# udaysankar01/xfeatSLAM

Measured on AMD Instinct MI355X. Metric: XFeat frames/s (VGA, 4096 kpts) + 4096x4096 desc-match pairs/s, higher is better.
Workload: dtype f32

## Files before the change

### include/xfeat_hip_bench.h

```cpp
#ifndef XFEAT_HIP_BENCH_H
#define XFEAT_HIP_BENCH_H

#include "xfeat_hip.h"

#ifdef __cplusplus
extern "C" {
#endif

enum {
    XFH_K_NONE = 0, XFH_K_MNN_GEMM = 1, XFH_K_CONV_MFMA = 2, XFH_K_CONV_DIRECT = 3,
    XFH_K_NMS = 4, XFH_K_SELECT = 5, XFH_K_DESC = 6, XFH_K_HEADS = 7, XFH_K_DIST_I32 = 8,
    XFH_K_PREPROC = 9, XFH_K_BEST2 = 10, XFH_K_DISTINCTIVE = 11, XFH_K_MNN_GEMM_SEG = 12,
    XFH_K_GRID_BUILD = 13, XFH_K_SEARCH_WINDOW = 14,
    XFH_K_FRAME_FINISH = 15, XFH_K_PROJ_CANDIDATES = 16, XFH_K_PROJ_RESOLVE = 17, XFH_K_PROJ_COUNT = 18, XFH_K_FUSE_SEARCH = 19,
    XFH_K_TRIANGULATION_SEARCH = 20, XFH_K_BOW_CANDIDATES = 21, XFH_K_BOW_RESOLVE = 22,
    XFH_K_MAPPROJ_CANDIDATES = 23, XFH_K_SIM3_SEARCH = 24, XFH_K_SIM3_AGREE = 25,
    XFH_K_INIT_CANDIDATES = 27, XFH_K_INIT_RESOLVE = 28, XFH_K_INIT_FINAL = 29,
    XFH_K_VOCAB_DESCEND = 31, XFH_K_VOCAB_FINISH = 32, XFH_K_BOWDB_SCORE = 33, XFH_K_BOWDB_SELECT = 34,
    XFH_K_POSE_OPTIMIZE = 35, XFH_K_COUNT = 36
};
int xfh_timing_enable(xfh_ctx* ctx, int kernel_id, unsigned layer_mask);
int xfh_timing_read(xfh_ctx* ctx, int* launches, double* total_ms);
int xfh_bench_mnn_gemm(xfh_ctx* ctx, const void* d_image1, int n1, const void* d_image2, int n2, int iters, double* us_per_launch);
int xfh_bench_match_prepared(xfh_ctx* ctx, const void* d_image1, int n1, const void* d_image2, int n2, float min_cossim,
                             int* d_idx1, int* d_idx2, float* d_dist, int* d_n_matches, int iters, double* us_per_call);
int xfh_bench_match_raw(xfh_ctx* ctx, const float* d_d1, int n1, const float* d_d2, int n2, float min_cossim,
                        int* d_idx1, int* d_idx2, float* d_dist, int* d_n_matches, int iters, double* us_per_call);
int xfh_bench_mnn_gemm_batch(xfh_ctx* ctx, int n_pairs, const void* const* d_image1, const int* n1, const void* const* d_image2, const int* n2,
                             int iters, double* us_per_launch, double* sclk_mhz);
int xfh_bench_match_batch(xfh_ctx* ctx, int n_pairs, const void* const* d_image1, const int* n1, const void* const* d_image2, const int* n2, float min_cossim,
                          int* const* d_idx1, int* const* d_idx2, float* const* d_dist, int* d_n_matches, int iters, double* us_per_call);
int xfh_debug_match_plan(int n_pairs, const int* n1, const int* n2, int num_cu, int* tiles, int* workgroups, int* tile0, int* planes_max, int* wg_lo,
                         unsigned long long* keys);
const char* xfh_kernel_name(int kernel_id);

enum {
    XFH_T_X = 0, XFH_T_XSTAT = 1, XFH_T_SKIP_POOL = 2,
    XFH_T_FEATS = 6, XFH_T_H1 = 8, XFH_T_K1H = 9,
    XFH_T_RAW0 = 16, XFH_T_STAT0 = 48, XFH_T_SEL = 80
};
int xfh_debug_tensor(xfh_ctx* ctx, int id, int frame, float* out, size_t capacity, size_t* count_out);

int xfh_debug_select(xfh_ctx* ctx, const unsigned long long* keys, int n, int width, int lap0, int lap1, int form,
                     unsigned long long* sel_out, int* n_out, int* hdr_out);


int xfh_bench_calib(xfh_ctx* ctx, int mode, size_t nbytes, int iters);
int xfh_bench_sclk(xfh_ctx* ctx, int mfmas, double* sclk_mhz, double* cycles_per_mfma);

#ifdef __cplusplus
}
#endif
#endif
```

### xfeatslam_amd/capi.py

```python
from __future__ import annotations

import ctypes as C
import os

import numpy as np

_DIR = os.path.dirname(os.path.abspath(__file__))
LIB_PATH = os.environ.get("XFEAT_HIP_LIB") or os.path.join(_DIR, "libxfeat_hip.so")
KNOBS_LIB_PATH = os.path.join(_DIR, "libxfeat_hip_knobs.so")

KP_DTYPE = np.dtype([("x", "<f4"), ("y", "<f4"), ("size", "<f4"), ("angle", "<f4"),
                     ("response", "<f4"), ("octave", "<i4"), ("class_id", "<i4")])
assert KP_DTYPE.itemsize == 28

OK = 0
STATUS = {0: "OK", 1: "INVALID_ARG", 2: "EMPTY_IMAGE", 3: "BAD_SIZE", 4: "NO_WEIGHTS", 5: "BAD_WEIGHTS",
          6: "HIP", 7: "NO_DEVICE", 8: "OUT_OF_MEMORY", 9: "BATCH_TOO_LARGE", 10: "IO", 11: "COMM"}
ERR_EMPTY_IMAGE = 2
ERR_NO_DEVICE = 7
ERR_COMM = 11

K = dict(NONE=0, MNN_GEMM=1, CONV_MFMA=2, CONV_DIRECT=3, NMS=4, SELECT=5, DESC=6, HEADS=7, DIST_I32=8, PREPROC=9, BEST2=10, DISTINCTIVE=11, MNN_GEMM_SEG=12, GRID_BUILD=13, SEARCH_WINDOW=14, FRAME_FINISH=15, PROJ_CANDIDATES=16, PROJ_RESOLVE=17, PROJ_COUNT=18, FUSE_SEARCH=19, TRIANGULATION_SEARCH=20, BOW_CANDIDATES=21, BOW_RESOLVE=22, MAPPROJ_CANDIDATES=23, SIM3_SEARCH=24, SIM3_AGREE=25, INIT_CANDIDATES=27, INIT_RESOLVE=28, INIT_FINAL=29, VOCAB_DESCEND=31, VOCAB_FINISH=32, BOWDB_SCORE=33, BOWDB_SELECT=34, POSE_OPTIMIZE=35)
T = dict(X=0, XSTAT=1, SKIP_POOL=2, FEATS=6, H1=8, K1H=9, RAW0=16, STAT0=48, SEL=80)


class Config(C.Structure):
    _fields_ = [("device", C.c_int32), ("max_height", C.c_int32), ("max_width", C.c_int32),
                ("nfeatures", C.c_int32), ("max_batch", C.c_int32), ("bn_mode", C.c_int32),
                ("nms_threshold", C.c_float), ("flags", C.c_int32), ("reserved", C.c_int32 * 7)]


class GridBounds(C.Structure):
    _fields_ = [("min_x", C.c_float), ("min_y", C.c_float), ("max_x", C.c_float), ("max_y", C.c_float)]


class Camera(C.Structure):
    _fields_ = [("fx", C.c_float), ("fy", C.c_float), ("cx", C.c_float), ("cy", C.c_float), ("k1", C.c_float), ("k2", C.c_float),
                ("p1", C.c_float), ("p2", C.c_float), ("k3", C.c_float), ("bf", C.c_float), ("width", C.c_int32), ("height", C.c_int32),
                ("reserved", C.c_int32 * 4)]


class Sim3Side(C.Structure):
    _fields_ = [("n", C.c_int), ("grid", C.c_void_p), ("kps", C.c_void_p), ("desc", C.c_void_p), ("desc_stride_bytes", C.c_size_t),
                ("points", C.c_void_p), ("dist", C.c_void_p), ("mp_desc", C.c_void_p), ("flags", C.c_void_p), ("Tw", C.c_void_p),
                ("status", C.c_void_p), ("match", C.c_void_p), ("best_dist", C.c_void_p), ("n_window", C.c_void_p), ("n_tested", C.c_void_p),
                ("level", C.c_void_p), ("proj_out", C.c_void_p)]
# ... 278 lines not shown
```

### xfeatslam_amd/csrc/capi_bench.cpp

```cpp
#include "capi_internal.h"
#include "mnn_seg_plan.h"
#include <stdlib.h>

template <typename F>
static int time_calls(xfh_ctx* c, int warmup, int iters, double* us_per_call, F call) {
    hipEvent_t e0, e1;
    HIPCK(c, hipEventCreate(&e0));
    if (hipEventCreate(&e1) != hipSuccess) { hipEventDestroy(e0); return XFH_ERR_HIP; }
    hipError_t e = hipSuccess;
    for (int i = 0; i < warmup && e == hipSuccess; ++i) e = call();
    if (e == hipSuccess) e = hipEventRecord(e0, c->stream);
    for (int i = 0; i < iters && e == hipSuccess; ++i) e = call();
    if (e == hipSuccess) e = hipEventRecord(e1, c->stream);
    if (e == hipSuccess) e = hipEventSynchronize(e1);
    float ms = 0.f;
    if (e == hipSuccess) e = hipEventElapsedTime(&ms, e0, e1);
    hipEventDestroy(e0); hipEventDestroy(e1);
    *us_per_call = (double)ms * 1e3 / iters;
    HIPCK(c, e);
    return XFH_OK;
}

extern "C" {

// ... 71 lines not shown
        tot += ms;
    }
    if (launches) *launches = t.nev;
    if (total_ms) *total_ms = tot;
    const bool overflow = t.dropped > 0;
    t.nev = 0; t.dropped = 0;
    return overflow ? XFH_ERR_BATCH_TOO_LARGE : XFH_OK;
}

int xfh_debug_tensor(xfh_ctx* c, int id, int frame, float* out, size_t cap, size_t* count_out) {
    if (!c || frame < 0 || frame >= c->B || !count_out) return XFH_ERR_INVALID_ARG;
    HIPCK(c, hipStreamSynchronize(c->stream));
    const size_t xs = (size_t)c->Hmax * c->Wmax;
    const int H = c->H, W = c->W, h8 = H / 8, w8 = W / 8, h4 = H / 4, w4 = W / 4;
    const float* src = nullptr; size_t n = 0;
    if (!was_written(c, id)) return XFH_ERR_INVALID_ARG;
    switch (id) {
        case XFH_T_X: src = c->X + frame * xs; n = (size_t)H * W; break;
        case XFH_T_XSTAT: src = c->xstat + frame * 2; n = 2; break;
        case XFH_T_SKIP_POOL: src = c->skip_pool + frame * (xs / 16); n = (size_t)h4 * w4; break;
        case XFH_T_FEATS: src = c->feats + frame * c->raw_stride[17]; n = (size_t)h8 * w8 * 64; break;
        case XFH_T_H1: src = c->H1 + frame * (xs / 64); n = (size_t)h8 * w8; break;
        case XFH_T_K1H: src = c->K1h + frame * xs; n = (size_t)H * W; break;
        default:
            if (id >= XFH_T_RAW0 && id < XFH_T_RAW0 + XFH_NUM_LAYERS) {
                const int i = id - XFH_T_RAW0;
                if (!c->raw[i]) return XFH_ERR_INVALID_ARG;
                src = c->raw[i] + frame * c->raw_stride[i]; n = (size_t)c->lh[i] * c->lw[i] * XFH_LAYERS[i].cout;
            } else if (id >= XFH_T_STAT0 && id < XFH_T_STAT0 + XFH_NUM_LAYERS) {
                const int i = id - XFH_T_STAT0;
                src = c->stat[i] + (size_t)frame * 2 * XFH_LAYERS[i].cout; n = 2 * (size_t)XFH_LAYERS[i].cout;
            } else if (id == XFH_T_SEL) {
                int N = 0;
                HIPCK(c, hipMemcpy(&N, c->sel_n + frame, sizeof(int), hipMemcpyDeviceToHost));
                *count_out = (size_t)N * 3;
                if (!out || cap < (size_t)N * 3) return out ? XFH_ERR_INVALID_ARG : XFH_OK;
                std::vector<u64> keys((size_t)N);
                if (N > 0) HIPCK(c, hipMemcpy(keys.data(), c->sel_key + (size_t)frame * c->cfg.nfeatures, (size_t)N * 8, hipMemcpyDeviceToHost));
                for (int i = 0; i < N; ++i) {
                    const unsigned idx = (unsigned)(keys[i] & 0xFFFFFFFFull);
                    out[i * 3 + 0] = (float)(idx % (unsigned)W); out[i * 3 + 1] = (float)(idx / (unsigned)W);
                    out[i * 3 + 2] = ord2f(~(unsigned)(keys[i] >> 32));
                }
                return XFH_OK;
            } else return XFH_ERR_INVALID_ARG;
    }
// ... 20 lines not shown
```

### xfeatslam_amd/csrc/kernels_conv.hip

```cpp
#include "ctx.h"
#include "heads_kp4.hip.h"
#include <stdlib.h>

struct ConvArgs {
    const float* in;
    StatSrc st;
    size_t in_stride;
    int Hin, Win;
    const float* w;
    const float* bias;
    float* out;
    size_t out_stride;
    int Hout, Wout;
    double* part;
    size_t part_stride;
    int tiles_x;
    const float* pool; size_t pool_stride; const float* skip_w; const float* skip_b;
    const float* r4; size_t s4; int H4, W4; StatSrc st4;
    const float* r5; size_t s5; int H5, W5; StatSrc st5;
    const float* xstat; const float* w0; const float* bias0;
    int dbg;
};

enum { PRO_PLAIN = 0, PRO_BN = 1, PRO_IN = 2, PRO_B2IN = 3, PRO_FUSE = 4, PRO_L0 = 5, PRO_UNFOLD = 6, PRO_FUSEA = 7  };
// ... 1187 lines not shown
    if constexpr (EPI == EPI_STATS) {
        sum += __shfl_xor(sum, 16); sq += __shfl_xor(sq, 16);
        sum += __shfl_xor(sum, 32); sq += __shfl_xor(sq, 32);
        double* s_red = (double*)smem;
        if (q == 0) { s_red[(pg * COUTW + cg * 16 + p) * 2] = sum; s_red[(pg * COUTW + cg * 16 + p) * 2 + 1] = sq; }
        __syncthreads();
        for (int co = t; co < COUTW; co += NTHR) {
            double S = 0.0, SS = 0.0;
#pragma unroll
            for (int m = 0; m < PGY; ++m) { S += s_red[(m * COUTW + co) * 2]; SS += s_red[(m * COUTW + co) * 2 + 1]; }
            double* pp = a.part + (size_t)b * a.part_stride + ((size_t)tile * COUT + co0 + co) * 2;
            pp[0] = S; pp[1] = SS;
        }
    }
    XFH_STAMP(a, 5);
}

enum { MID_BIAS_STORE = 0 , MID_BIAS_RELU = 1  };
struct ChainArgs {
    ConvArgs a;
    const float* w1; const float* bias1;
    const float* w2; const float* bias2;
    float* mid_out; size_t mid_stride;
};
template <int NL, int WM, int PRO, int MID0, int EPI, bool SSTAT = false>
__global__ __launch_bounds__(64 * WM)
void k_chain1x1(ChainArgs ca, int ntile, int total) {
    constexpr int CIN = 64, COUT = 64, NT = 2, WW = 16, WH = 2, TH = WM * WH, TW = WW;
    constexpr int NTHR = 64 * WM, COUTP = 64, CP = CIN + 4, WS = CIN + 4, G = CIN / 8;
    constexpr int NITEM = TH * TW * G, NIT = (NITEM + NTHR - 1) / NTHR;
    constexpr int IN_FLOATS = TH * TW * CP, W_FLOATS = COUTP * WS;
    static_assert(NTHR % G == 0 && NIT <= 32, "staging");
    const ConvArgs& a = ca.a;

    extern __shared__ __attribute__((aligned(16))) float smem[];
    float* s_in = smem;
    float* s_w = smem + IN_FLOATS;
    double* s_red = (double*)(s_w + NL * W_FLOATS);
    float* s_stat = (float*)(s_red + WM * COUTP * 2);
    static_assert(!SSTAT || sizeof(double) * 512 <= sizeof(float) * IN_FLOATS, "bn_fold scratch in the input tile");
    int stat_b = -1;

    const int t = threadIdx.x;
    {
        const float* ws[3] = {a.w, ca.w1, ca.w2};
#pragma unroll
        for (int l = 0; l < NL; ++l)
            for (int f = t; f < COUTP * (CIN / 4); f += NTHR) {
// ... 83 lines not shown
                    for (int j = 0; j < 4; ++j)
                        acc[n] = __builtin_amdgcn_mfma_f32_32x32x2f32(av[j], bv[j], acc[n], 0, 0, 0);
                }
            }
            if (l == NL - 1) break;
            const bool store_mid = l == 0 && MID0 == MID_BIAS_STORE;
            if (store_mid) {
                double dsum[NT], dsq[NT];
                float* wave_out = ca.mid_out + (size_t)b * ca.mid_stride + ((size_t)oy0 * a.Wout + tx0) * COUT;
                conv_epilogue<COUT, NT, WW, WH, EPI_BIAS>(acc, wave_out, a.Wout, a.Hout - oy0, a.Wout - tx0, i, h, bias0, dsum, dsq);
            } else {
                XFH_MFMA_SETTLE();
            }
#pragma unroll
            for (int n = 0; n < NT; ++n) {
                const int c = n * 32 + i;
                const int pos = (c & ~7) + 4 * (c & 1) + ((c & 7) >> 1);
                const float bv = l == 0 ? bias0[n] : bias1[n];
#pragma unroll
                for (int r = 0; r < 16; ++r) {
                    float v = acc[n][r] + bv;
                    if (!store_mid) v = fmaxf(v, 0.f);
                    mid_row[((r & 3) + 8 * (r >> 2)) * CP + pos] = v;
                }
            }
        }

        double sum[NT], sq[NT];
        {
            float* wave_out = a.out + (size_t)b * a.out_stride + ((size_t)oy0 * a.Wout + tx0) * COUT;
            conv_epilogue<COUT, NT, WW, WH, EPI>(acc, wave_out, a.Wout, a.Hout - oy0, a.Wout - tx0, i, h, biasl, sum, sq);
        }
        if constexpr (EPI == EPI_STATS) {
#pragma unroll
            for (int n = 0; n < NT; ++n) {
                sum[n] += __shfl_xor(sum[n], 32);
                sq[n] += __shfl_xor(sq[n], 32);
                if (h == 0) {
                    const int co = n * 32 + i;
                    s_red[(wm * COUTP + co) * 2 + 0] = sum[n];
                    s_red[(wm * COUTP + co) * 2 + 1] = sq[n];
                }
            }
        }
        __syncthreads();
        if constexpr (EPI == EPI_STATS) {
// ... 342 lines not shown
        default: return hipErrorInvalidValue;
    }
}

hipError_t launch_basic_layer(xfh_ctx* c, int li, const float* in, size_t in_stride, int src, int pro, int Hin, int Win, int B) {
    if (c->cfg.bn_mode == XFH_BN_RUNNING_FOLDED) return launch_basic_layer_t<EPI_BIAS_RELU>(c, li, in, in_stride, src, pro, Hin, Win, B);
    return launch_basic_layer_t<EPI_STATS>(c, li, in, in_stride, src, pro, Hin, Win, B);
}

hipError_t launch_block1_stats(xfh_ctx* c, const StatSrc& xs, int H, int W, int B) {
    const int np = conv_layer_npart(0, H, W);
    c->lh[0] = H; c->lw[0] = W; c->npart[0] = np;
    const size_t xsz = (size_t)c->Hmax * c->Wmax;
    launch_k(c, XFH_K_CONV_DIRECT, 0, k_block1_stats, dim3(np, 1, B), dim3(256), 0, (const float*)c->X, xsz, xs, H, W,
             (W + L0S_TW - 1) / L0S_TW, (const float*)c->w.direct[0], c->part[0], c->part_stride[0], c->skip_pool, xsz / 16);
    hipError_t e = hipGetLastError();
    mark_written(c, XFH_T_SKIP_POOL);
    if (e != hipSuccess || consumer_fold(B)) return e;
    hipLaunchKernelGGL(k_bn_finalize, dim3(B), dim3(256), 0, c->stream, (const double*)c->part[0], c->part_stride[0], np, 4, (double)H * (double)W, c->stat[0]);
    mark_written(c, XFH_T_STAT0);
    return hipGetLastError();
}

template <int NL, int WM, int PRO, int MID0, int EPI, bool SSTAT = false>
static hipError_t chain_launch(xfh_ctx* c, const ChainArgs& ca, int B, int* npart_out, int layer) {
    constexpr int TH = 2 * WM, TW = 16;
    constexpr size_t LDS = sizeof(float) * ((size_t)TH * TW * 68 + (size_t)NL * 64 * 68 + (SSTAT ? 128 : 0)) + sizeof(double) * WM * 64 * 2;
    static_assert(LDS <= 160 * 1024, "LDS budget");
    ChainArgs aa = ca;
    aa.a.tiles_x = (ca.a.Wout + TW - 1) / TW;
    const int ntile = aa.a.tiles_x * ((ca.a.Hout + TH - 1) / TH);
    if (npart_out) *npart_out = ntile;
    auto kern = k_chain1x1<NL, WM, PRO, MID0, EPI, SSTAT>;
    XFH_SET_LDS_ATTR_ONCE(c, kern, LDS);
    const int total = ntile * B;
    const int per_cu = (int)((160 * 1024) / LDS);
    const int grid = total < 256 * per_cu ? total : 256 * per_cu;
    launch_k(c, XFH_K_CONV_MFMA, layer, kern, dim3(grid), dim3(64 * WM), LDS, aa, ntile, total);
    return hipGetLastError();
}

hipError_t launch_fusion_chain(xfh_ctx* c, int Hh, int Wh, int B, int* done) {
    *done = 0;
    const bool folded = c->cfg.bn_mode == XFH_BN_RUNNING_FOLDED;
    ChainArgs ca{};
    ConvArgs& a = ca.a;
    a.in = c->raw[17]; a.st = stat_src(c, 17, B); a.in_stride = c->raw_stride[17]; a.Hin = Hh; a.Win = Wh; a.Hout = Hh; a.Wout = Wh;
    a.w = c->w.fus2; a.bias = c->w.fus2_bias;
    ca.mid_out = c->feats; ca.mid_stride = c->raw_stride[17];
    ca.w1 = c->w.mfma[18];
    int np = 0;
    hipError_t e;
    if (!persistent(B) && folded) {
        ca.bias1 = c->w.bn_bias[18]; ca.w2 = c->w.mfma[19]; ca.bias2 = c->w.bn_bias[19];
        a.out = c->raw[19]; a.out_stride = c->raw_stride[19];
        e = chain_launch<3, 4, PRO_BN, MID_BIAS_STORE, EPI_BIAS_RELU>(c, ca, B, &np, 19);
        if (e != hipSuccess) return e;
        mark_written(c, XFH_T_FEATS); mark_written(c, XFH_T_RAW0 + 19);
        c->lh[18] = Hh; c->lw[18] = Wh; c->npart[18] = np; c->lh[19] = Hh; c->lw[19] = Wh; c->npart[19] = np;
        *done = 2;
        return hipSuccess;
    }
    if (consumer_fold(B)) {
        a.out = c->raw[18]; a.out_stride = c->raw_stride[18]; a.part = c->part[18]; a.part_stride = c->part_stride[18];
        e = chain_launch<2, 4, PRO_BN, MID_BIAS_STORE, EPI_STATS, true>(c, ca, B, &np, 18);
        if (e != hipSuccess) return e;
        mark_written(c, XFH_T_FEATS); mark_written(c, XFH_T_RAW0 + 18);
        c->lh[18] = Hh; c->lw[18] = Wh; c->npart[18] = np;
        *done = 1;
        return hipSuccess;
    }
    if (!folded) {
        a.out = c->raw[18]; a.out_stride = c->raw_stride[18]; a.part = c->part[18]; a.part_stride = c->part_stride[18];
        e = chain_launch<2, 4, PRO_BN, MID_BIAS_STORE, EPI_STATS>(c, ca, B, &np, 18);
        if (e != hipSuccess) return e;
        mark_written(c, XFH_T_FEATS); mark_written(c, XFH_T_RAW0 + 18);
        c->lh[18] = Hh; c->lw[18] = Wh; c->npart[18] = np;
        *done = 1;
        if (c->cfg.bn_mode == XFH_BN_BATCH_STATS) {
            hipLaunchKernelGGL(k_bn_finalize, dim3(B), dim3(256), 0, c->stream, (const double*)c->part[18], c->part_stride[18], np, 64, (double)Hh * (double)Wh, c->stat[18]);
            mark_written(c, XFH_T_STAT0 + 18);
        }
        return hipGetLastError();
    }
    ca.bias1 = c->w.bn_bias[18];
    a.out = c->raw[18]; a.out_stride = c->raw_stride[18];
    e = chain_launch<2, 4, PRO_BN, MID_BIAS_STORE, EPI_BIAS_RELU>(c, ca, B, &np, 18);
    if (e != hipSuccess) return e;
    mark_written(c, XFH_T_FEATS); mark_written(c, XFH_T_RAW0 + 18);
    c->lh[18] = Hh; c->lw[18] = Wh; c->npart[18] = np;
    *done = 1;
    return hipSuccess;
}

hipError_t launch_finalize_image(xfh_ctx* c, int B, int npart, double count) {
    hipLaunchKernelGGL(k_bn_finalize, dim3(B), dim3(256), 0, c->stream, (const double*)c->pre_part,
                       (size_t)c->pre_npart * 2, npart, 1, count, c->xstat);
    mark_written(c, XFH_T_XSTAT);
    return hipGetLastError();
}
```

### xfeatslam_amd/csrc/kernels_misc.hip

```cpp
#include "ctx.h"
#include "mnn_layout.h"
#include "heads_kp4.hip.h"
#include <stdlib.h>

__device__ __forceinline__ double wave_sum(double v) {
    v += __shfl_xor(v, 32); v += __shfl_xor(v, 16); v += __shfl_xor(v, 8);
    v += __shfl_xor(v, 4); v += __shfl_xor(v, 2); v += __shfl_xor(v, 1);
    return v;
}

__device__ __forceinline__ void lin_coeff(int in, int out, int d, int& i0, int& i1, float& l0, float& l1) {
    const float scale = (float)in / (float)out;
    float src = fmaf(scale, (float)d + 0.5f, -0.5f);
    if (src < 0.f) src = 0.f;
    int a = (int)src;
    if (a > in - 1) a = in - 1;
    float lam = src - (float)a;
    lam = fminf(fmaxf(lam, 0.f), 1.f);
    i0 = a; i1 = a + ((a < in - 1) ? 1 : 0);
    l1 = lam; l0 = 1.f - lam;
}

__device__ __forceinline__ float grid_coord(int pos, int full, int size) {
    const float g = 2.0f * ((float)pos / (float)(full - 1)) - 1.0f;
// ... 80 lines not shown
    f32x4 rv[16];
    {
        const float* rp = rawH + (size_t)b * raw_stride;
#pragma unroll
        for (int k = 0; k < 16; ++k) {
            const int item = t + k * HF_PX, lp = item >> 4, g = item & 15;
            rv[k] = *(const f32x4*)(rp + (size_t)min(p0 + lp, npix - 1) * 64 + g * 4);
        }
    }
    stage_stat(sH, b, 64, blockIdx.x == 0, st, (double*)sA, t, HF_PX);
#pragma unroll
    for (int k = 0; k < 16; ++k) {
        const int item = t + k * HF_PX, lp = item >> 4, g = item & 15;
#pragma unroll
        for (int j = 0; j < 4; ++j) sA[(g * 4 + j) * HF_LD + lp] = fmaxf(fmaf(rv[k][j], st[64 + g * 4 + j], st[g * 4 + j]), 0.f);
    }
    __syncthreads();
    float acc = 0.f;
    for (int k = 0; k < 64; ++k) acc = fmaf(sA[k * HF_LD + t], wh[k], acc);
    acc += bh[0];
    if (pix < npix) H1[(size_t)b * h1_stride + pix] = 1.0f / (1.0f + xfh_expf(0.f - acc));
}

__global__ __launch_bounds__(HF_PX)
void k_heads_kp(const float* __restrict__ rawK, StatSrc sK,
                size_t raw_stride, const float* __restrict__ wk , const float* __restrict__ bk ,
                int Hh, int Wh, float* __restrict__ K1h, size_t k1h_stride) {
    __shared__ float sA[64 * HF_LD];
    __shared__ float st[128];
    const int t = threadIdx.x, b = blockIdx.z;
    const int npix = Hh * Wh, p0 = blockIdx.x * HF_PX;
    const int pix = p0 + t;
    f32x4 rv[16];
    {
        const float* rp = rawK + (size_t)b * raw_stride;
#pragma unroll
        for (int k = 0; k < 16; ++k) {
            const int item = t + k * HF_PX, lp = item >> 4, g = item & 15;
            rv[k] = *(const f32x4*)(rp + (size_t)min(p0 + lp, npix - 1) * 64 + g * 4);
        }
    }
    stage_stat(sK, b, 64, blockIdx.x == 0, st, (double*)sA, t, HF_PX);
#pragma unroll
    for (int k = 0; k < 16; ++k) {
        const int item = t + k * HF_PX, lp = item >> 4, g = item & 15;
#pragma unroll
        for (int j = 0; j < 4; ++j) sA[(g * 4 + j) * HF_LD + lp] = fmaxf(fmaf(rv[k][j], st[64 + g * 4 + j], st[g * 4 + j]), 0.f);
    }
    __syncthreads();
    float acc[65];
#pragma unroll
    for (int n = 0; n < 65; ++n) acc[n] = 0.f;
#pragma unroll 2
    for (int k = 0; k < 64; ++k) {
        const float a = sA[k * HF_LD + t];
        const XFH_CONST float* wr = (const XFH_CONST float*)wk + k * 68;
#pragma unroll
        for (int n = 0; n < 65; ++n) acc[n] = fmaf(a, wr[n], acc[n]);
    }
    float mx = -__builtin_huge_valf();
#pragma unroll
    for (int n = 0; n < 65; ++n) { acc[n] += bk[n]; mx = fmaxf(mx, acc[n]); }
    float sum = 0.f;
#pragma unroll
    for (int n = 0; n < 65; ++n) { acc[n] = xfh_expf(acc[n] - mx); sum += acc[n]; }
    const Recip ks = recip_of(sum);
    if (pix < npix) {
        const int y = pix / Wh, x = pix % Wh;
        float* o = K1h + (size_t)b * k1h_stride + (size_t)(8 * y) * (8 * Wh) + 8 * x;
#pragma unroll
        for (int i = 0; i < 8; ++i) {
            *(f32x4*)(o + (size_t)i * 8 * Wh) = f32x4{div_by(acc[i * 8], ks), div_by(acc[i * 8 + 1], ks), div_by(acc[i * 8 + 2], ks), div_by(acc[i * 8 + 3], ks)};
            *(f32x4*)(o + (size_t)i * 8 * Wh + 4) = f32x4{div_by(acc[i * 8 + 4], ks), div_by(acc[i * 8 + 5], ks), div_by(acc[i * 8 + 6], ks), div_by(acc[i * 8 + 7], ks)};
        }
    }
}

__global__ __launch_bounds__(4 * HK4_PX)
void k_heads_kp4(Kp4Args k) {
    __shared__ __attribute__((aligned(16))) float smem_kp4[HK4_LDS_FLOATS];
    heads_kp4_body(k, blockIdx.x, blockIdx.z, smem_kp4);
}

__device__ __forceinline__ void feat_norm_px(const float* __restrict__ feats, size_t m_stride, int npix, float* __restrict__ nrm, size_t n_stride, int b, int p) {
    if (p >= npix) return;
    const float* m = feats + (size_t)b * m_stride + (size_t)p * 64;
    double ss = 0.0;
#pragma unroll
    for (int g = 0; g < 16; ++g) {
        const f32x4 v = *(const f32x4*)(m + g * 4);
#pragma unroll
        for (int q = 0; q < 4; ++q) ss = fma((double)v[q], (double)v[q], ss);
    }
    nrm[(size_t)b * n_stride + p] = fmaxf((float)sqrt(ss), 1e-12f);
}
__global__ __launch_bounds__(256)
void k_feat_norm(const float* __restrict__ feats, size_t m_stride, int npix, float* __restrict__ nrm, size_t n_stride) {
    feat_norm_px(feats, m_stride, npix, nrm, n_stride, blockIdx.z, blockIdx.x * 256 + threadIdx.x);
}

#define NMS_TW 64
#define NMS_TH 16
#define NMS_LD 72
#define NMS_HCW (NMS_TW / 8 + 2)
#define NMS_HCH (NMS_TH / 8 + 2)
#define NMS_HC (NMS_HCW * NMS_HCH)
template <bool HEAT>
__global__ __launch_bounds__(256)
void k_nms_score(const float* __restrict__ K1h, size_t k_stride, const float* __restrict__ H1, size_t h_stride,
                 int H, int W, float thr, u64* __restrict__ cand, size_t cand_cap, int* __restrict__ cand_count,
                 int nms_blocks, const float* __restrict__ fn_feats, size_t fn_m_stride, int fn_npix, float* __restrict__ fn_nrm, size_t fn_n_stride,
                 const float* __restrict__ rawH, StatSrc sH, size_t raw_stride, const float* __restrict__ wh, const float* __restrict__ bh, float* __restrict__ H1out) {
    __shared__ __attribute__((aligned(16))) float s[(NMS_TH + 4) * NMS_LD];
    __shared__ u64 keys[1024];
    __shared__ unsigned short cpx[1024];
    __shared__ int cnt, base;
    __shared__ float s_act[HEAT ? NMS_HC * 65 : 1];
    __shared__ float s_hst[HEAT ? 128 : 1];
    __shared__ float s_h1[HEAT ? NMS_HC : 1];
    const int t = threadIdx.x, b = blockIdx.z;
    if ((int)blockIdx.x >= nms_blocks) {
// ... 595 lines not shown
                            mark_written(c, XFH_T_XSTAT); }
    else CK(launch_finalize_image(c, B, npre, (double)H * (double)W));
    if (c->cfg.bn_mode == XFH_BN_BATCH_STATS) CK(launch_block1_stats(c, xsrc, H, W, B));
    else {
        hipLaunchKernelGGL(k_norm_aux, dim3((h4 * w4 + 255) / 256, 1, B), dim3(256), 0, s, c->X, xs, xsrc, H, W, c->skip_pool, xs / 16);
        CK(hipGetLastError());
        mark_written(c, XFH_T_SKIP_POOL);
    }
    const bool ride = ride_mode(c, B);
    if (!ride) {
        const bool two = !(c->cfg.flags & XFH_FLAG_SERIAL_BRANCH);
        hipStream_t branch = two ? c->aux_stream : s;
        hipError_t e = hipEventRecord(c->ev_fork, s);
        if (e == hipSuccess) e = hipStreamWaitEvent(branch, c->ev_fork, 0);
        CK(e);
        c->stream = branch;
        e = launch_basic_layer(c, 20, c->X, xs, -1, PRO_UNFOLD, h8, w8, B);
        if (e == hipSuccess) e = launch_basic_layer(c, 21, c->raw[20], c->raw_stride[20], 20, PRO_BN, h8, w8, B);
        if (e == hipSuccess) e = launch_basic_layer(c, 22, c->raw[21], c->raw_stride[21], 21, PRO_BN, h8, w8, B);
        if (e == hipSuccess) {
            if (consumer_fold(B))
                launch_k(c, XFH_K_HEADS, -1, k_heads_kp4, dim3((h8 * w8 + HK4_PX - 1) / HK4_PX, 1, B), dim3(4 * HK4_PX), 0,
                         Kp4Args{(const float*)c->raw[22], stat_src(c, 22, B), c->raw_stride[22], (const float*)c->w.kp3_w, (const float*)c->w.kp3_b, h8, w8, c->K1h, xs});
            else
            launch_k(c, XFH_K_HEADS, -1, k_heads_kp, dim3((h8 * w8 + HF_PX - 1) / HF_PX, 1, B), dim3(HF_PX), 0,
                     (const float*)c->raw[22], stat_src(c, 22, B), c->raw_stride[22], (const float*)c->w.kp3_w, (const float*)c->w.kp3_b, h8, w8, c->K1h, xs);
            e = hipGetLastError();
            mark_written(c, XFH_T_K1H);
        }
        c->stream = s;
        const hipError_t e2 = hipEventRecord(c->ev_join, branch);
        if (e != hipSuccess || e2 != hipSuccess) { hipStreamSynchronize(branch); return e != hipSuccess ? e : e2; }
    }
    auto backbone = [&]() -> hipError_t {
    CK(launch_basic_layer(c, 1, c->X, xs, 0, PRO_L0, H, W, B));
    CK(launch_basic_layer(c, 2, c->raw[1], c->raw_stride[1], 1, PRO_BN, c->lh[1], c->lw[1], B));
    if (ride) {
        CK(launch_layer_with_rider(c, 3, c->raw[2], c->raw_stride[2], 2, PRO_BN, c->lh[2], c->lw[2], B, c->K1h, xs));
        CK(launch_layer_with_rider(c, 4, c->raw[3], c->raw_stride[3], 3, PRO_B2IN, h4, w4, B, c->K1h, xs));
        CK(launch_layer_with_rider(c, 5, c->raw[4], c->raw_stride[4], 4, PRO_BN, h4, w4, B, c->K1h, xs));
        CK(launch_layer_with_rider(c, 6, c->raw[5], c->raw_stride[5], 5, PRO_BN, h4, w4, B, c->K1h, xs));
        mark_written(c, XFH_T_K1H);
    } else {
    CK(launch_basic_layer(c, 3, c->raw[2], c->raw_stride[2], 2, PRO_BN, c->lh[2], c->lw[2], B));
    CK(launch_basic_layer(c, 4, c->raw[3], c->raw_stride[3], 3, PRO_B2IN, h4, w4, B));
    CK(launch_basic_layer(c, 5, c->raw[4], c->raw_stride[4], 4, PRO_BN, h4, w4, B));
    CK(launch_basic_layer(c, 6, c->raw[5], c->raw_stride[5], 5, PRO_BN, h4, w4, B));
    }
    CK(launch_basic_layer(c, 7, c->raw[6], c->raw_stride[6], 6, PRO_BN, h8, w8, B));
// ... 16 lines not shown
                       (const float*)c->raw[19], stat_src(c, 19, B), c->raw_stride[19], (const float*)c->w.heat2_w, (const float*)c->w.heat2_b, h8 * w8, c->H1, xs / 64);
    mark_written(c, XFH_T_H1);
    return hipGetLastError();
    };
    {
        const hipError_t eb = backbone();
        const hipError_t ej = ride ? hipSuccess : hipStreamWaitEvent(s, c->ev_join, 0);
        CK(eb); CK(ej);
    }
    const int nms_blocks = ((W + NMS_TW - 1) / NMS_TW) * ((H + NMS_TH - 1) / NMS_TH);
    const int fn_blocks = consumer_fold(B) ? (h8 * w8 + 255) / 256 : 0;
    if (fn_blocks && !c->no_nms_heat) {
        mark_written(c, XFH_T_H1);
        launch_k(c, XFH_K_NMS, -1, k_nms_score<true>, dim3(nms_blocks + fn_blocks, 1, B), dim3(256), 0, c->K1h, xs, c->H1, xs / 64,
                       H, W, c->cfg.nms_threshold, c->cand, c->cand_cap, c->cand_count,
                       nms_blocks, (const float*)c->feats, c->raw_stride[17], h8 * w8, c->feat_nrm, xs / 64,
                       fn_blocks ? (const float*)c->raw[19] : (const float*)nullptr, stat_src(c, 19, B), c->raw_stride[19], (const float*)c->w.heat2_w, (const float*)c->w.heat2_b, c->H1);
    } else
        launch_k(c, XFH_K_NMS, -1, k_nms_score<false>, dim3(nms_blocks + fn_blocks, 1, B), dim3(256), 0, c->K1h, xs, c->H1, xs / 64,
                       H, W, c->cfg.nms_threshold, c->cand, c->cand_cap, c->cand_count,
                       nms_blocks, (const float*)c->feats, c->raw_stride[17], h8 * w8, c->feat_nrm, xs / 64,
                       fn_blocks ? (const float*)c->raw[19] : (const float*)nullptr, stat_src(c, 19, B), c->raw_stride[19], (const float*)c->w.heat2_w, (const float*)c->w.heat2_b, c->H1);
    CK(hipGetLastError());
    if (nf <= SEL_FAST_MAX) {
        XFH_SET_LDS_ATTR_ONCE(c, k_select, SEL_LDS_BYTES);
        launch_k(c, XFH_K_SELECT, -1, k_select, dim3(B), dim3(1024), SEL_LDS_BYTES, (const u64*)c->cand, c->cand_cap, (const int*)c->cand_count, W, nf,
                 lap0, lap1, rw, c->slot_src, c->sel_key, c->sel_n, d_records, rec, c->select_legacy ? 1 : 0);
    } else {
        XFH_SET_LDS_ATTR_ONCE(c, k_select_generic, SEL_LDS_KEYS * 8);
        launch_k(c, XFH_K_SELECT, -1, k_select_generic, dim3(B), dim3(1024), SEL_LDS_KEYS * 8, c->cand, c->cand_cap, (const int*)c->cand_count, W, nf,
                 lap0, lap1, rw, c->slot_src, c->sel_key, c->sel_n, d_records, rec);
    }
    CK(hipGetLastError());
    mark_written(c, XFH_T_SEL);
    if (!fn_blocks) {
        hipLaunchKernelGGL(k_feat_norm, dim3((h8 * w8 + 255) / 256, 1, B), dim3(256), 0, s, (const float*)c->feats, c->raw_stride[17], h8 * w8, c->feat_nrm, xs / 64);
        CK(hipGetLastError());
    }
    const int dslots = d_images ? (nf + MNN_PANEL - 1) / MNN_PANEL * MNN_PANEL : nf;
    launch_k(c, XFH_K_DESC, -1, k_desc, dim3((dslots + 15) / 16, 1, B), dim3(256), 0, c->feats, c->raw_stride[17], (const float*)c->feat_nrm, xs / 64, c->slot_src, c->sel_key, H, W, nf, rw, rh,
                       d_records, rec, xfh_record_kps_offset(), xfh_record_desc_offset(nf), write_padding ? 1 : 0,
             d_images, (size_t)(dslots / MNN_PANEL) * MNN_PANEL_FLOATS);
    return hipGetLastError();
}

#define HIPCK(c, x) do { hipError_t _e = (x); if (_e != hipSuccess) { (c)->hip_err = std::string(#x) + ": " + hipGetErrorString(_e); return XFH_ERR_HIP; } } while (0)
extern "C" int xfh_debug_select(xfh_ctx* c, const unsigned long long* keys, int n, int width, int lap0, int lap1, int form, unsigned long long* sel_out, int* n_out, int* hdr_out) {
    if (!c || !keys || n < 0 || (size_t)n > c->cand_cap || width <= 0 || !sel_out || !n_out || !hdr_out || c->cfg.nfeatures > SEL_FAST_MAX) return XFH_ERR_INVALID_ARG;
    HIPCK(c, hipSetDevice(c->cfg.device));
    const int nf = c->cfg.nfeatures;
    const size_t rec = xfh_record_bytes(nf);
    HIPCK(c, hipMemcpyAsync(c->cand, keys, sizeof(u64) * (size_t)n, hipMemcpyHostToDevice, c->stream));
    HIPCK(c, hipMemcpyAsync(c->cand_count, &n, sizeof(int), hipMemcpyHostToDevice, c->stream));
    XFH_SET_LDS_ATTR_ONCE(c, k_select, SEL_LDS_BYTES);
    const int legacy = form == 0 ? (c->select_legacy ? 1 : 0) : (form == 2 ? 1 : 0);
    hipLaunchKernelGGL(k_select, dim3(1), dim3(1024), SEL_LDS_BYTES, c->stream, (const u64*)c->cand, c->cand_cap, (const int*)c->cand_count, width, nf,
                       lap0, lap1, 1.0f, c->slot_src, c->sel_key, c->sel_n, c->d_records, rec, legacy);
    HIPCK(c, hipGetLastError());
    HIPCK(c, hipMemcpyAsync(n_out, c->sel_n, sizeof(int), hipMemcpyDeviceToHost, c->stream));
    HIPCK(c, hipMemcpyAsync(hdr_out, c->d_records, 4 * sizeof(int), hipMemcpyDeviceToHost, c->stream));
    HIPCK(c, hipStreamSynchronize(c->stream));
// ... 6 lines not shown
```

Measured before the change: 31890.

## Fuse descriptor norm into chain1x1 epilogue and move keypoint head to MFMA

The per-pixel descriptor L2 norm is now computed in the chain1x1 kernel that writes the descriptor features, which removes the separate k_feat_norm launch and its extra read of the feature map. The keypoint head kernel is rewritten as a persistent, wave-tiled kernel: 32x32x2 f32 MFMA handles the 64 logit channels, the dustbin channel is done with scalar FMAs, and the next tile's loads are prefetched while the current one computes. This trades a simple per-thread FMA loop for more complex LDS layouts and lane shuffles. The new norm path relies on the feats data held in LDS matching what was written out, and the nms fused-norm path (fn_blocks) may now compute the norm twice.

After: 32310, median of 6. +1.3%, better.

```diff
diff --git a/include/xfeat_hip_bench.h b/include/xfeat_hip_bench.h
--- a/include/xfeat_hip_bench.h
+++ b/include/xfeat_hip_bench.h
@@ -36,7 +36,7 @@
 
 enum {
     XFH_T_X = 0, XFH_T_XSTAT = 1, XFH_T_SKIP_POOL = 2,
-    XFH_T_FEATS = 6, XFH_T_H1 = 8, XFH_T_K1H = 9,
+    XFH_T_FEATS = 6, XFH_T_M1N = 7, XFH_T_H1 = 8, XFH_T_K1H = 9,
     XFH_T_RAW0 = 16, XFH_T_STAT0 = 48, XFH_T_SEL = 80
 };
 int xfh_debug_tensor(xfh_ctx* ctx, int id, int frame, float* out, size_t capacity, size_t* count_out);
diff --git a/xfeatslam_amd/capi.py b/xfeatslam_amd/capi.py
--- a/xfeatslam_amd/capi.py
+++ b/xfeatslam_amd/capi.py
@@ -21,7 +21,7 @@
 ERR_COMM = 11
 
 K = dict(NONE=0, MNN_GEMM=1, CONV_MFMA=2, CONV_DIRECT=3, NMS=4, SELECT=5, DESC=6, HEADS=7, DIST_I32=8, PREPROC=9, BEST2=10, DISTINCTIVE=11, MNN_GEMM_SEG=12, GRID_BUILD=13, SEARCH_WINDOW=14, FRAME_FINISH=15, PROJ_CANDIDATES=16, PROJ_RESOLVE=17, PROJ_COUNT=18, FUSE_SEARCH=19, TRIANGULATION_SEARCH=20, BOW_CANDIDATES=21, BOW_RESOLVE=22, MAPPROJ_CANDIDATES=23, SIM3_SEARCH=24, SIM3_AGREE=25, INIT_CANDIDATES=27, INIT_RESOLVE=28, INIT_FINAL=29, VOCAB_DESCEND=31, VOCAB_FINISH=32, BOWDB_SCORE=33, BOWDB_SELECT=34, POSE_OPTIMIZE=35)
-T = dict(X=0, XSTAT=1, SKIP_POOL=2, FEATS=6, H1=8, K1H=9, RAW0=16, STAT0=48, SEL=80)
+T = dict(X=0, XSTAT=1, SKIP_POOL=2, FEATS=6, M1N=7, H1=8, K1H=9, RAW0=16, STAT0=48, SEL=80)
 
 
 class Config(C.Structure):
diff --git a/xfeatslam_amd/csrc/capi_bench.cpp b/xfeatslam_amd/csrc/capi_bench.cpp
--- a/xfeatslam_amd/csrc/capi_bench.cpp
+++ b/xfeatslam_amd/csrc/capi_bench.cpp
@@ -117,6 +117,18 @@
         case XFH_T_FEATS: src = c->feats + frame * c->raw_stride[17]; n = (size_t)h8 * w8 * 64; break;
         case XFH_T_H1: src = c->H1 + frame * (xs / 64); n = (size_t)h8 * w8; break;
         case XFH_T_K1H: src = c->K1h + frame * xs; n = (size_t)H * W; break;
+        case XFH_T_M1N: {
+            n = (size_t)h8 * w8 * 64;
+            *count_out = n;
+            if (!out) return XFH_OK;
+            if (cap < n) return XFH_ERR_INVALID_ARG;
+            std::vector<float> nrm((size_t)h8 * w8);
+            HIPCK(c, hipMemcpy(out, c->feats + frame * c->raw_stride[17], n * sizeof(float), hipMemcpyDeviceToHost));
+            HIPCK(c, hipMemcpy(nrm.data(), c->feat_nrm + frame * (xs / 64), nrm.size() * sizeof(float), hipMemcpyDeviceToHost));
+            for (size_t p = 0; p < nrm.size(); ++p)
+                for (int ch = 0; ch < 64; ++ch) out[p * 64 + ch] = out[p * 64 + ch] / nrm[p];
+            return XFH_OK;
+        }
         default:
             if (id >= XFH_T_RAW0 && id < XFH_T_RAW0 + XFH_NUM_LAYERS) {
                 const int i = id - XFH_T_RAW0;
diff --git a/xfeatslam_amd/csrc/kernels_conv.hip b/xfeatslam_amd/csrc/kernels_conv.hip
--- a/xfeatslam_amd/csrc/kernels_conv.hip
+++ b/xfeatslam_amd/csrc/kernels_conv.hip
@@ -1233,8 +1233,9 @@
     const float* w1; const float* bias1;
     const float* w2; const float* bias2;
     float* mid_out; size_t mid_stride;
+    float* nrm; size_t nrm_stride;
 };
-template <int NL, int WM, int PRO, int MID0, int EPI, bool SSTAT = false>
+template <int NL, int WM, int PRO, int MID0, int EPI, bool SSTAT = false, bool FNRM = false>
 __global__ __launch_bounds__(64 * WM)
 void k_chain1x1(ChainArgs ca, int ntile, int total) {
     constexpr int CIN = 64, COUT = 64, NT = 2, WW = 16, WH = 2, TH = WM * WH, TW = WW;
@@ -1364,6 +1365,26 @@
                     float v = acc[n][r] + bv;
                     if (!store_mid) v = fmaxf(v, 0.f);
                     mid_row[((r & 3) + 8 * (r >> 2)) * CP + pos] = v;
+                }
+            }
+            if constexpr (FNRM && MID0 == MID_BIAS_STORE) {
+                if (l == 0) {
+                    __builtin_amdgcn_fence(__ATOMIC_ACQ_REL, "wavefront");
+                    if (h == 0) {
+                        const float* row = s_in + (wm * 32 + i) * CP;
+                        double ss = 0.0;
+#pragma unroll
+                        for (int kk = 0; kk < CIN / 8; ++kk) {
+                            const f32x4 ev = *(const f32x4*)(row + kk * 8), od = *(const f32x4*)(row + kk * 8 + 4);
+#pragma unroll
+                            for (int j = 0; j < 4; ++j) {
+                                ss = fma((double)ev[j], (double)ev[j], ss);
+                                ss = fma((double)od[j], (double)od[j], ss);
+                            }
+                        }
+                        const int oy = oy0 + i / WW, ox = tx0 + i % WW;
+                        if (oy < a.Hout && ox < a.Wout) ca.nrm[(size_t)b * ca.nrm_stride + (size_t)oy * a.Wout + ox] = fmaxf((float)sqrt(ss), 1e-12f);
+                    }
                 }
             }
         }
@@ -1752,7 +1773,7 @@
     return hipGetLastError();
 }
 
-template <int NL, int WM, int PRO, int MID0, int EPI, bool SSTAT = false>
+template <int NL, int WM, int PRO, int MID0, int EPI, bool SSTAT = false, bool FNRM = false>
 static hipError_t chain_launch(xfh_ctx* c, const ChainArgs& ca, int B, int* npart_out, int layer) {
     constexpr int TH = 2 * WM, TW = 16;
     constexpr size_t LDS = sizeof(float) * ((size_t)TH * TW * 68 + (size_t)NL * 64 * 68 + (SSTAT ? 128 : 0)) + sizeof(double) * WM * 64 * 2;
@@ -1761,7 +1782,7 @@
     aa.a.tiles_x = (ca.a.Wout + TW - 1) / TW;
     const int ntile = aa.a.tiles_x * ((ca.a.Hout + TH - 1) / TH);
     if (npart_out) *npart_out = ntile;
-    auto kern = k_chain1x1<NL, WM, PRO, MID0, EPI, SSTAT>;
+    auto kern = k_chain1x1<NL, WM, PRO, MID0, EPI, SSTAT, FNRM>;
     XFH_SET_LDS_ATTR_ONCE(c, kern, LDS);
     const int total = ntile * B;
     const int per_cu = (int)((160 * 1024) / LDS);
@@ -1778,6 +1799,7 @@
     a.in = c->raw[17]; a.st = stat_src(c, 17, B); a.in_stride = c->raw_stride[17]; a.Hin = Hh; a.Win = Wh; a.Hout = Hh; a.Wout = Wh;
     a.w = c->w.fus2; a.bias = c->w.fus2_bias;
     ca.mid_out = c->feats; ca.mid_stride = c->raw_stride[17];
+    ca.nrm = c->feat_nrm; ca.nrm_stride = (size_t)c->Hmax * c->Wmax / 64;
     ca.w1 = c->w.mfma[18];
     int np = 0;
     hipError_t e;
@@ -1802,7 +1824,7 @@
     }
     if (!folded) {
         a.out = c->raw[18]; a.out_stride = c->raw_stride[18]; a.part = c->part[18]; a.part_stride = c->part_stride[18];
-        e = chain_launch<2, 4, PRO_BN, MID_BIAS_STORE, EPI_STATS>(c, ca, B, &np, 18);
+        e = chain_launch<2, 4, PRO_BN, MID_BIAS_STORE, EPI_STATS, false, true>(c, ca, B, &np, 18);
         if (e != hipSuccess) return e;
         mark_written(c, XFH_T_FEATS); mark_written(c, XFH_T_RAW0 + 18);
         c->lh[18] = Hh; c->lw[18] = Wh; c->npart[18] = np;
@@ -1815,7 +1837,7 @@
     }
     ca.bias1 = c->w.bn_bias[18];
     a.out = c->raw[18]; a.out_stride = c->raw_stride[18];
-    e = chain_launch<2, 4, PRO_BN, MID_BIAS_STORE, EPI_BIAS_RELU>(c, ca, B, &np, 18);
+    e = chain_launch<2, 4, PRO_BN, MID_BIAS_STORE, EPI_BIAS_RELU, false, true>(c, ca, B, &np, 18);
     if (e != hipSuccess) return e;
     mark_written(c, XFH_T_FEATS); mark_written(c, XFH_T_RAW0 + 18);
     c->lh[18] = Hh; c->lw[18] = Wh; c->npart[18] = np;
diff --git a/xfeatslam_amd/csrc/kernels_misc.hip b/xfeatslam_amd/csrc/kernels_misc.hip
--- a/xfeatslam_amd/csrc/kernels_misc.hip
+++ b/xfeatslam_amd/csrc/kernels_misc.hip
@@ -126,59 +126,140 @@
     if (pix < npix) H1[(size_t)b * h1_stride + pix] = 1.0f / (1.0f + xfh_expf(0.f - acc));
 }
 
-__global__ __launch_bounds__(HF_PX)
+#define HKM_PX 128
+#define HKM_CP 68
+#define HKM_WG_PER_CU 3
+__global__ __launch_bounds__(256)
 void k_heads_kp(const float* __restrict__ rawK, StatSrc sK,
                 size_t raw_stride, const float* __restrict__ wk , const float* __restrict__ bk ,
-                int Hh, int Wh, float* __restrict__ K1h, size_t k1h_stride) {
-    __shared__ float sA[64 * HF_LD];
-    __shared__ float st[128];
-    const int t = threadIdx.x, b = blockIdx.z;
-    const int npix = Hh * Wh, p0 = blockIdx.x * HF_PX;
-    const int pix = p0 + t;
-    f32x4 rv[16];
-    {
-        const float* rp = rawK + (size_t)b * raw_stride;
-#pragma unroll
-        for (int k = 0; k < 16; ++k) {
-            const int item = t + k * HF_PX, lp = item >> 4, g = item & 15;
-            rv[k] = *(const f32x4*)(rp + (size_t)min(p0 + lp, npix - 1) * 64 + g * 4);
-        }
-    }
-    stage_stat(sK, b, 64, blockIdx.x == 0, st, (double*)sA, t, HF_PX);
-#pragma unroll
-    for (int k = 0; k < 16; ++k) {
-        const int item = t + k * HF_PX, lp = item >> 4, g = item & 15;
-#pragma unroll
-        for (int j = 0; j < 4; ++j) sA[(g * 4 + j) * HF_LD + lp] = fmaxf(fmaf(rv[k][j], st[64 + g * 4 + j], st[g * 4 + j]), 0.f);
-    }
-    __syncthreads();
-    float acc[65];
-#pragma unroll
-    for (int n = 0; n < 65; ++n) acc[n] = 0.f;
-#pragma unroll 2
-    for (int k = 0; k < 64; ++k) {
-        const float a = sA[k * HF_LD + t];
-        const XFH_CONST float* wr = (const XFH_CONST float*)wk + k * 68;
-#pragma unroll
-        for (int n = 0; n < 65; ++n) acc[n] = fmaf(a, wr[n], acc[n]);
-    }
-    float mx = -__builtin_huge_valf();
-#pragma unroll
-    for (int n = 0; n < 65; ++n) { acc[n] += bk[n]; mx = fmaxf(mx, acc[n]); }
-    float sum = 0.f;
-#pragma unroll
-    for (int n = 0; n < 65; ++n) { acc[n] = xfh_expf(acc[n] - mx); sum += acc[n]; }
-    const Recip ks = recip_of(sum);
-    if (pix < npix) {
-        const int y = pix / Wh, x = pix % Wh;
-        float* o = K1h + (size_t)b * k1h_stride + (size_t)(8 * y) * (8 * Wh) + 8 * x;
-#pragma unroll
-        for (int i = 0; i < 8; ++i) {
-            *(f32x4*)(o + (size_t)i * 8 * Wh) = f32x4{div_by(acc[i * 8], ks), div_by(acc[i * 8 + 1], ks), div_by(acc[i * 8 + 2], ks), div_by(acc[i * 8 + 3], ks)};
-            *(f32x4*)(o + (size_t)i * 8 * Wh + 4) = f32x4{div_by(acc[i * 8 + 4], ks), div_by(acc[i * 8 + 5], ks), div_by(acc[i * 8 + 6], ks), div_by(acc[i * 8 + 7], ks)};
-        }
-    }
-}
+                int Hh, int Wh, float* __restrict__ K1h, size_t k1h_stride, int nblk, int total) {
+    __shared__ __attribute__((aligned(16))) float s_w[64 * HKM_CP];
+    __shared__ __attribute__((aligned(16))) float s_a[HKM_PX * HKM_CP];
+    const int t = threadIdx.x;
+    const int wave = __builtin_amdgcn_readfirstlane(t >> 6), lane = t & 63, i = lane & 31, h = lane >> 5, g = lane & 7;
+    const int npix = Hh * Wh;
+#pragma unroll
+    for (int q = 0; q < 4; ++q) {
+        const int f = t + q * 256, k = f >> 4, nq = f & 15;
+        const f32x4 w = *(const f32x4*)(wk + k * 68 + nq * 4);
+        const int pos = (k & ~7) + 4 * (k & 1) + ((k & 7) >> 1);
+#pragma unroll
+        for (int j = 0; j < 4; ++j) s_w[(nq * 4 + j) * HKM_CP + pos] = w[j];
+    }
+    const float wd = wk[lane * 68 + 64];
+    const float bias0 = bk[i], bias1 = bk[32 + i], biasd = bk[64];
+    __syncthreads();
+
+    float* const rows = s_a + wave * 32 * HKM_CP;
+    f32x4 v0[4], v1[4], sm0, sm1, sr0, sr1;
+    auto load_tile = [&](int tile) {
+        const int b = tile / nblk, p0 = (tile - b * nblk) * HKM_PX + wave * 32;
+        const float* rp = rawK + (size_t)b * raw_stride + g * 8;
+#pragma unroll
+        for (int q = 0; q < 4; ++q) {
+            const float* p = rp + (size_t)min(p0 + (lane >> 3) + q * 8, npix - 1) * 64;
+            v0[q] = *(const f32x4*)p; v1[q] = *(const f32x4*)(p + 4);
+        }
+        const float* st = sK.stat + (size_t)b * 128 + g * 8;
+        sm0 = *(const f32x4*)st; sm1 = *(const f32x4*)(st + 4); sr0 = *(const f32x4*)(st + 64); sr1 = *(const f32x4*)(st + 68);
+    };
+    auto store_tile = [&]() {
+#pragma unroll
+        for (int q = 0; q < 4; ++q) {
+            f32x4 x0 = v0[q], x1 = v1[q];
+#pragma unroll
+            for (int c = 0; c < 4; ++c) {
+                x0[c] = fmaxf(fmaf(x0[c], sr0[c], sm0[c]), 0.f);
+                x1[c] = fmaxf(fmaf(x1[c], sr1[c], sm1[c]), 0.f);
+            }
+            float* d = rows + ((lane >> 3) + q * 8) * HKM_CP + g * 8;
+            *(f32x4*)d = f32x4{x0.x, x0.z, x1.x, x1.z};
+            *(f32x4*)(d + 4) = f32x4{x0.y, x0.w, x1.y, x1.w};
+        }
+    };
+
+    int tile = blockIdx.x;
+    load_tile(tile);
+    while (true) {
+        const int b = tile / nblk, p0 = (tile - b * nblk) * HKM_PX + wave * 32;
+        store_tile();
+        const int next = tile + gridDim.x;
+        const bool has_next = next < total;
+        if (has_next) load_tile(next);
+        __builtin_amdgcn_fence(__ATOMIC_ACQ_REL, "wavefront");
+        if (p0 < npix) {
+            f32x16 acc[2];
+#pragma unroll
+            for (int n = 0; n < 2; ++n)
+#pragma unroll
+                for (int r = 0; r < 16; ++r) acc[n][r] = 0.f;
+            float accd = 0.f;
+            const float* pa = rows + i * HKM_CP;
+            const float* pw = s_w + i * HKM_CP + 4 * h;
+#pragma unroll
+            for (int kk = 0; kk < 8; ++kk) {
+                const f32x4 a0 = *(const f32x4*)(pa + kk * 8), a1 = *(const f32x4*)(pa + kk * 8 + 4);
+                const f32x4 b0 = *(const f32x4*)(pw + kk * 8), b1 = *(const f32x4*)(pw + 32 * HKM_CP + kk * 8);
+#pragma unroll
+                for (int j = 0; j < 4; ++j) {
+                    const float av = h ? a1[j] : a0[j];
+                    acc[0] = __builtin_amdgcn_mfma_f32_32x32x2f32(av, b0[j], acc[0], 0, 0, 0);
+                    acc[1] = __builtin_amdgcn_mfma_f32_32x32x2f32(av, b1[j], acc[1], 0, 0, 0);
+                }
+#pragma unroll
+                for (int j = 0; j < 4; ++j) {
+                    accd = fmaf(a0[j], __builtin_bit_cast(float, __builtin_amdgcn_readlane(__builtin_bit_cast(int, wd), kk * 8 + 2 * j)), accd);
+                    accd = fmaf(a1[j], __builtin_bit_cast(float, __builtin_amdgcn_readlane(__builtin_bit_cast(int, wd), kk * 8 + 2 * j + 1)), accd);
+                }
+            }
+            XFH_MFMA_SETTLE();
+            {
+                float* lrow = rows + 4 * h * HKM_CP + i;
+#pragma unroll
+                for (int n = 0; n < 2; ++n)
+#pragma unroll
+                    for (int r = 0; r < 16; ++r) lrow[((r & 3) + 8 * (r >> 2)) * HKM_CP + n * 32] = acc[n][r] + (n ? bias1 : bias0);
+            }
+            __builtin_amdgcn_fence(__ATOMIC_ACQ_REL, "wavefront");
+            float lg[32];
+#pragma unroll
+            for (int q = 0; q < 8; ++q) {
+                const f32x4 v = *(const f32x4*)(rows + i * HKM_CP + 32 * h + q * 4);
+                lg[q * 4] = v.x; lg[q * 4 + 1] = v.y; lg[q * 4 + 2] = v.z; lg[q * 4 + 3] = v.w;
+            }
+            const float ld = accd + biasd;
+            float mx = ld;
+#pragma unroll
+            for (int n = 0; n < 32; ++n) mx = fmaxf(mx, lg[n]);
+            mx = fmaxf(mx, __shfl_xor(mx, 32));
+#pragma unroll
+            for (int n = 0; n < 32; ++n) lg[n] = xfh_expf(lg[n] - mx);
+            const float ed = xfh_expf(ld - mx);
+            float s0 = 0.f;
+#pragma unroll
+            for (int n = 0; n < 32; ++n) s0 += lg[n];
+            float s1 = __shfl(s0, i);
+#pragma unroll
+            for (int n = 0; n < 32; ++n) s1 += lg[n];
+            s1 += ed;
+            const Recip ks = recip_of(__shfl(s1, 32 + i));
+            const int pix = p0 + i;
+            if (pix < npix) {
+                const int y = pix / Wh, x = pix % Wh;
+                float* o = K1h + (size_t)b * k1h_stride + (size_t)(8 * y + 4 * h) * (8 * Wh) + 8 * x;
+#pragma unroll
+                for (int r = 0; r < 4; ++r) {
+                    *(f32x4*)(o + (size_t)r * 8 * Wh) = f32x4{div_by(lg[r * 8], ks), div_by(lg[r * 8 + 1], ks), div_by(lg[r * 8 + 2], ks), div_by(lg[r * 8 + 3], ks)};
+                    *(f32x4*)(o + (size_t)r * 8 * Wh + 4) = f32x4{div_by(lg[r * 8 + 4], ks), div_by(lg[r * 8 + 5], ks), div_by(lg[r * 8 + 6], ks), div_by(lg[r * 8 + 7], ks)};
+                }
+            }
+            __builtin_amdgcn_fence(__ATOMIC_ACQ_REL, "wavefront");
+        }
+        if (!has_next) break;
+        tile = next;
+    }
+}
+
 
 __global__ __launch_bounds__(4 * HK4_PX)
 void k_heads_kp4(Kp4Args k) {
@@ -197,10 +278,6 @@
         for (int q = 0; q < 4; ++q) ss = fma((double)v[q], (double)v[q], ss);
     }
     nrm[(size_t)b * n_stride + p] = fmaxf((float)sqrt(ss), 1e-12f);
-}
-__global__ __launch_bounds__(256)
-void k_feat_norm(const float* __restrict__ feats, size_t m_stride, int npix, float* __restrict__ nrm, size_t n_stride) {
-    feat_norm_px(feats, m_stride, npix, nrm, n_stride, blockIdx.z, blockIdx.x * 256 + threadIdx.x);
 }
 
 #define NMS_TW 64
@@ -842,9 +919,11 @@
             if (consumer_fold(B))
                 launch_k(c, XFH_K_HEADS, -1, k_heads_kp4, dim3((h8 * w8 + HK4_PX - 1) / HK4_PX, 1, B), dim3(4 * HK4_PX), 0,
                          Kp4Args{(const float*)c->raw[22], stat_src(c, 22, B), c->raw_stride[22], (const float*)c->w.kp3_w, (const float*)c->w.kp3_b, h8, w8, c->K1h, xs});
-            else
-            launch_k(c, XFH_K_HEADS, -1, k_heads_kp, dim3((h8 * w8 + HF_PX - 1) / HF_PX, 1, B), dim3(HF_PX), 0,
-                     (const float*)c->raw[22], stat_src(c, 22, B), c->raw_stride[22], (const float*)c->w.kp3_w, (const float*)c->w.kp3_b, h8, w8, c->K1h, xs);
+            else {
+                const int nblk = (h8 * w8 + HKM_PX - 1) / HKM_PX, total = nblk * B;
+                launch_k(c, XFH_K_HEADS, -1, k_heads_kp, dim3(total < 256 * HKM_WG_PER_CU ? total : 256 * HKM_WG_PER_CU), dim3(256), 0,
+                         (const float*)c->raw[22], stat_src(c, 22, B), c->raw_stride[22], (const float*)c->w.kp3_w, (const float*)c->w.kp3_b, h8, w8, c->K1h, xs, nblk, total);
+            }
             e = hipGetLastError();
             mark_written(c, XFH_T_K1H);
         }
@@ -907,6 +986,7 @@
                        nms_blocks, (const float*)c->feats, c->raw_stride[17], h8 * w8, c->feat_nrm, xs / 64,
                        fn_blocks ? (const float*)c->raw[19] : (const float*)nullptr, stat_src(c, 19, B), c->raw_stride[19], (const float*)c->w.heat2_w, (const float*)c->w.heat2_b, c->H1);
     CK(hipGetLastError());
+    mark_written(c, XFH_T_M1N);
     if (nf <= SEL_FAST_MAX) {
         XFH_SET_LDS_ATTR_ONCE(c, k_select, SEL_LDS_BYTES);
         launch_k(c, XFH_K_SELECT, -1, k_select, dim3(B), dim3(1024), SEL_LDS_BYTES, (const u64*)c->cand, c->cand_cap, (const int*)c->cand_count, W, nf,
@@ -918,10 +998,6 @@
     }
     CK(hipGetLastError());
     mark_written(c, XFH_T_SEL);
-    if (!fn_blocks) {
-        hipLaunchKernelGGL(k_feat_norm, dim3((h8 * w8 + 255) / 256, 1, B), dim3(256), 0, s, (const float*)c->feats, c->raw_stride[17], h8 * w8, c->feat_nrm, xs / 64);
-        CK(hipGetLastError());
-    }
     const int dslots = d_images ? (nf + MNN_PANEL - 1) / MNN_PANEL * MNN_PANEL : nf;
     launch_k(c, XFH_K_DESC, -1, k_desc, dim3((dslots + 15) / 16, 1, B), dim3(256), 0, c->feats, c->raw_stride[17], (const float*)c->feat_nrm, xs / 64, c->slot_src, c->sel_key, H, W, nf, rw, rh,
                        d_records, rec, xfh_record_kps_offset(), xfh_record_desc_offset(nf), write_padding ? 1 : 0,
```
